# nitishthatte/QuadrotorILQR

Measured on AMD Instinct MI355X. Metric: iLQR solves/sec (batch, 100-knot SE(3) quadrotor), higher is better.
Workload: dtype f64

## Files before the change

### quadrotorilqr_amd/csrc/host/api_calls.h

```cpp
#pragma once

extern "C" {
int qilqr_solve_batch_device(qilqr_solver *s, const double *d_init, const double *d_desired_batch, int32_t B,
                             int32_t n, double *d_out_traj, double *d_out_cost, int32_t *d_out_status,
                             int32_t *d_out_iters, int32_t *d_out_n_bwd, int32_t *d_out_n_fwd) {
  return solve_batch_device_impl(s, d_init, d_desired_batch, B, n, d_out_traj, d_out_cost, d_out_status, d_out_iters,
                                 d_out_n_bwd, d_out_n_fwd, true);
}

int qilqr_stream_wait_event(qilqr_solver *s, void *hip_event) {
  if (!s || !hip_event) return fail(QILQR_ERR_INVALID_ARG, "null argument");
  HIP_TRY(hipSetDevice(s->device));
  HIP_TRY(hipStreamWaitEvent(s->stream, (hipEvent_t)hip_event, 0));
  return QILQR_OK;
}

namespace {
bool pinned_or_null(const void *p) {
  if (!p) return true;
  hipPointerAttribute_t a;
  if (hipPointerGetAttributes(&a, p) != hipSuccess) {
    (void)hipGetLastError();
    return false;
  }
// ... 68 lines not shown
    if (out_traj) e = hipMemcpyAsync(out_traj, s->stage_traj, tb, hipMemcpyDeviceToHost, s->stream);
    if (e == hipSuccess && out_cost) e = hipMemcpyAsync(out_cost, d_cost, sizeof(double) * B, hipMemcpyDeviceToHost, s->stream);
    if (e == hipSuccess && out_status) e = hipMemcpyAsync(out_status, d_int, sizeof(int) * B, hipMemcpyDeviceToHost, s->stream);
    if (e == hipSuccess && out_iters) e = hipMemcpyAsync(out_iters, d_int + B, sizeof(int) * B, hipMemcpyDeviceToHost, s->stream);
    if (e == hipSuccess && out_n_bwd) e = hipMemcpyAsync(out_n_bwd, d_int + 2 * B, sizeof(int) * B, hipMemcpyDeviceToHost, s->stream);
    if (e == hipSuccess && out_n_fwd) e = hipMemcpyAsync(out_n_fwd, d_int + 3 * B, sizeof(int) * B, hipMemcpyDeviceToHost, s->stream);
    if (e == hipSuccess) e = hipStreamSynchronize(s->stream);
    if (e == hipSuccess) e = hipGetLastError();
  }
  if (s->dev.profile) drain_events(s);
  if (e != hipSuccess) return fail(QILQR_ERR_HIP, std::string("copy back: ") + hipGetErrorString(e));
  return device_error(s);
}

void *qilqr_host_alloc(size_t bytes) {
  void *p = nullptr;
  if (hipHostMalloc(&p, bytes ? bytes : 1, hipHostMallocDefault) != hipSuccess) {
    g_last_error = "hipHostMalloc failed";
    return nullptr;
  }
  return p;
}
void qilqr_host_free(void *p) {
  if (p) (void)hipHostFree(p);
}

int qilqr_solve(qilqr_solver *s, const double *init, int32_t n, double *out_traj, double *out_cost,
                int32_t *out_status, int32_t *out_iters, double *debug_cost, double *debug_trajs,
                int32_t debug_cap, int32_t *n_debug) {
  if (!s || !init || !out_traj) return fail(QILQR_ERR_INVALID_ARG, "null argument");
  if (n <= 0) return fail(QILQR_ERR_INVALID_ARG, "empty trajectory");
  int rc;
  if ((rc = check_quaternions(init, n, "initial trajectory"))) return rc;
  if ((rc = begin_batch(s, 1, n, nullptr, E_SOLVE))) return rc;
  if ((rc = upload_tiled(s, init, s->st.traj[0], 1, n, 18))) return rc;
  const bool want_debug = s->options.populate_debug && debug_cap > 0 && (debug_cost || debug_trajs);
  if (want_debug) {
    const size_t want_t = debug_trajs ? (size_t)debug_cap * n * 18 : 0, want_c = (size_t)debug_cap;
    if (want_t > s->dbg_traj_cap) {
      if (s->dbg_trajs) (void)hipFree(s->dbg_trajs);
      s->dbg_trajs = nullptr;
      s->dbg_traj_cap = 0;
      HIP_TRY(hipMalloc((void **)&s->dbg_trajs, sizeof(double) * want_t));
      s->dbg_traj_cap = want_t;
    }
    if (want_c > s->dbg_cost_cap) {
      if (s->dbg_cost) (void)hipFree(s->dbg_cost);
      s->dbg_cost = nullptr;
      s->dbg_cost_cap = 0;
      HIP_TRY(hipMalloc((void **)&s->dbg_cost, sizeof(double) * want_c));
      s->dbg_cost_cap = want_c;
    }
    if (!s->dbg_seen) HIP_TRY(hipMalloc((void **)&s->dbg_seen, sizeof(int)));
    HIP_TRY(hipMemsetAsync(s->dbg_seen, 0, sizeof(int), s->stream));
    s->st.dbg_trajs = debug_trajs ? s->dbg_trajs : nullptr;
    s->st.dbg_cost = s->dbg_cost;
    s->st.dbg_seen = s->dbg_seen;
    s->st.dbg_cap = (int)debug_cap;
  }
  struct DebugRingScope {
    qilqr_solver *s;
    ~DebugRingScope() { s->st.dbg_trajs = s->st.dbg_cost = nullptr; s->st.dbg_seen = nullptr; s->st.dbg_cap = 0; }
  } ring_scope{s};
  auto capture = [&]() -> int {
    if (!want_debug || s->round_captured) return QILQR_OK;
    if (s->f32)
      launch(s, K_OTHER, k_debug_capture<float>, dim3(1), dim3(256), s->st, (int)n, debug_trajs ? s->dbg_trajs : nullptr, s->dbg_cost, s->dbg_seen, (int)debug_cap);
    else
// ... 118 lines not shown
```

### quadrotorilqr_amd/csrc/host/batch_solve.h

```cpp
#pragma once

namespace {
constexpr int MAX_TRACKED_DEVICES = 64;
std::atomic<int> g_solves_in_flight[MAX_TRACKED_DEVICES];
struct InFlight {
  std::atomic<int> &n;
  explicit InFlight(int device) : n(g_solves_in_flight[(unsigned)device % MAX_TRACKED_DEVICES]) { n.fetch_add(1, std::memory_order_relaxed); }
  ~InFlight() { n.fetch_sub(1, std::memory_order_relaxed); }
  bool alone(bool always = false) const { return always || n.load(std::memory_order_relaxed) == 1; }
};

int wait_for_count(const unsigned long long *word, hipStream_t stream, long old, unsigned long long *v) {
  const unsigned tag = (unsigned)((old & 0x3fffffff) + 1);
  for (long spins = 0;; ++spins) {
    *v = __atomic_load_n(word, __ATOMIC_ACQUIRE);
    if ((unsigned)(*v >> 32) == tag) return QILQR_OK;
    if ((spins & 1023) == 1023) {
      const hipError_t q = hipStreamQuery(stream);
      if (q != hipErrorNotReady) {
        *v = __atomic_load_n(word, __ATOMIC_ACQUIRE);
        if ((unsigned)(*v >> 32) == tag) return QILQR_OK;
        return fail(QILQR_ERR_HIP, std::string("a round never reported its active count: ") + hipGetErrorString(q));
      }
    }
// ... 62 lines not shown

int fire_early_out(qilqr_solver *s, long B, long n, EarlyOut *eo, unsigned active) {
  eo->fired = true;
  eo->late_cap = (int)active;
  *eo->layout = late_layout((long)active, n);
  int *early = s->d_early, *late_count = (int *)(s->d_late + eo->layout->count);
  launch(s, K_OTHER, k_mark_final, dim3(cdiv(B, 256)), dim3(256), s->st, (int)B, early, late_count);
  HIP_TRY(hipEventRecord(s->early_evt, s->stream));
  HIP_TRY(hipStreamWaitEvent(s->early_stream, s->early_evt, 0));
  hipStream_t main_stream = s->stream;
  s->stream = s->early_stream;
  int *d_int = s->stage_int;
  const int rc = gather(s, B, n, eo->h_traj ? s->stage_traj : nullptr, eo->h_cost ? s->stage_cost : nullptr, eo->h_status ? d_int : nullptr,
                        eo->h_iters ? d_int + B : nullptr, eo->h_bwd ? d_int + 2 * B : nullptr, eo->h_fwd ? d_int + 3 * B : nullptr, early, 1,
                        nullptr);
  s->stream = main_stream;
  if (rc) return rc;
  hipStream_t es = s->early_stream;
  if (eo->h_traj) HIP_TRY(hipMemcpyAsync(eo->h_traj, s->stage_traj, sizeof(double) * 18 * (size_t)B * n, hipMemcpyDeviceToHost, es));
  if (eo->h_cost) HIP_TRY(hipMemcpyAsync(eo->h_cost, s->stage_cost, sizeof(double) * B, hipMemcpyDeviceToHost, es));
  if (eo->h_status) HIP_TRY(hipMemcpyAsync(eo->h_status, d_int, sizeof(int) * B, hipMemcpyDeviceToHost, es));
  if (eo->h_iters) HIP_TRY(hipMemcpyAsync(eo->h_iters, d_int + B, sizeof(int) * B, hipMemcpyDeviceToHost, es));
  if (eo->h_bwd) HIP_TRY(hipMemcpyAsync(eo->h_bwd, d_int + 2 * B, sizeof(int) * B, hipMemcpyDeviceToHost, es));
  if (eo->h_fwd) HIP_TRY(hipMemcpyAsync(eo->h_fwd, d_int + 3 * B, sizeof(int) * B, hipMemcpyDeviceToHost, es));
  HIP_TRY(hipEventRecord(s->early_done, es));
  return QILQR_OK;
}

template <typename F>
int run_solve(qilqr_solver *s, long B, long n, int sync_every, F on_round, bool drain = true,
              const std::function<int(unsigned)> *on_count = nullptr, bool double_ok = false) {
  int rc;
  s->round_captured = false;
  if ((rc = launch_linearize(s, B, n, 0, 0))) return rc;
  {
    launch(s, K_OTHER, k_init, dim3(cdiv(B, 64)), dim3(64), s->params, s->st, (int)B, (int)n);
  }
  if (!(0.0 < s->params.max_iters)) {
    HIP_TRY(hipStreamSynchronize(s->stream));
    return QILQR_OK;
  }
  const double bound = (std::fmin(s->params.max_iters, 1e7) + 1.0) * ((double)std::max(s->params.ls_max_iters, 1) + 1.0) * (1.0 + max_restarts(s->params));
  const long max_rounds = (long)std::fmin(bound, 2e9);
  const int lag = (sync_every > 1) ? std::min(sync_every, 6) : 0;
  if (lag == 0) {
    for (long round = 0; round < max_rounds; ++round) {
      if ((rc = launch_backward(s, B, n, 0))) return rc;
      int active = 0;
      if ((rc = read_active(s, &active))) return rc;
      if ((rc = on_round())) return rc;
      if (active == 0) break;
      if ((rc = launch_rollout(s, B, n, F_SEARCH, round))) return rc;
      if ((rc = launch_linearize(s, B, n, 1, F_SEARCH))) return rc;
    }
  } else {
    struct CounterSet {
      qilqr_solver *s;
      int *base;
      CounterSet(qilqr_solver *s_, long round, bool two) : s(s_), base(s_->st.counters) { if (two) s->st.counters = base + (round & 1) * COUNT_WORDS; }
      ~CounterSet() { s->st.counters = base; }
    };
    for (int k = 0; k < 8; ++k) s->h_active[k] = 0;
    const InFlight in_flight(s->device);
    const bool can_fuse = s->route.combined && !s->compact;
    const TailFuse tf = tail_fuse(s->route, s->compact, 1);
    if (s->compact) s->plan_heads.push_back(0);
    unsigned seen_active = (unsigned)B;
    long used = B;
    bool pending_publish = false;
    unsigned launched_rounds[8] = {1, 1, 1, 1, 1, 1, 1, 1};
    bool two_sets = false;
    bool tail_started = false;
    for (long round = 0; round < max_rounds; ++round) {
      const RoctxRange range(s, "round", round);
      const bool compacting = s->compact && !tail_started && (seen_active > tf.stop || (tf.kinds && used > tf.slots));
      if (s->compact && tf.kinds && !compacting && used <= tf.slots && round >= tf.from) tail_started = true;
      s->live_hint = (long)seen_active;
      const bool fuse_now = (can_fuse || tail_started) && in_flight.alone(s->dev.fuse_in_flight == 1);
      if (fuse_now && s->route.round_kernel) {
        const RoundForm f = round_form(s->route, (can_fuse || tail_started) && double_ok, true, seen_active, used);
        if ((rc = launch_round(s, used, n, round, pending_publish, f.rounds, f.six))) return rc;
        s->round_captured = true;
        launched_rounds[round & 7] = f.rounds;
        pending_publish = true;
        two_sets = true;
        if ((rc = on_round())) return rc;
        goto round_enqueued;
      }
      if (pending_publish) {
        launch(s, K_OTHER, k_publish_active, dim3(1), dim3(64), s->st.counters + ((round + 1) & 1) * COUNT_WORDS, s->st.host_active,
               (int)((round - 1) & 0x3fffffff));
        pending_publish = false;
      }
      launched_rounds[round & 7] = 1;
      s->round_captured = false;
      {
      const CounterSet counter_set(s, round, two_sets);
      if (fuse_now) {
        if ((rc = launch_backward_rollout(s, used, n))) return rc;
      } else {
        if ((rc = launch_backward(s, used, n, 0))) return rc;
        if (compacting) {
          if ((rc = launch_compact(s, used, n))) return rc;
          used = slots_in_use(used, seen_active);
        }
        if ((rc = launch_rollout(s, used, n, F_SEARCH, round))) return rc;
      }
      if ((rc = on_round())) return rc;
      if ((rc = launch_linearize(s, used, n, 1, F_SEARCH, (int)(round & 0x3fffffff)))) return rc;
      }
    round_enqueued:
      if (round >= lag) {
        const long old = round - lag;
        unsigned long long v;
        if ((rc = wait_for_count(&s->h_active[old & 7], s->stream, old, &v))) return rc;
        if ((unsigned)v == 0) break;
        const unsigned now_at_most = ((unsigned)v + launched_rounds[old & 7] - 1) / launched_rounds[old & 7];
        seen_active = now_at_most;
        if (__atomic_load_n(s->h_active + 8 * (1 + qilqr_solver::MAX_PARTS), __ATOMIC_ACQUIRE)) {
          (void)hipStreamSynchronize(s->stream);
          if (s->early_stream) (void)hipStreamSynchronize(s->early_stream);
          return device_error(s);
        }
        if (on_count && (rc = (*on_count)(now_at_most))) return rc;
      }
    }
  }
  if (drain) {
    HIP_TRY(hipStreamSynchronize(s->stream));
    HIP_TRY(hipGetLastError());
    return device_error(s);
  }
  return QILQR_OK;
}

struct Part {
  hipStream_t stream;
  BatchState st;
  long nb;
  unsigned long long *h_active;
  bool done;
  unsigned seen_active;
  long used;
  bool tail = false;
  bool round_kernel = false;
  unsigned launched_rounds[8] = {1, 1, 1, 1, 1, 1, 1, 1};
};
BatchState slice_state(const qilqr_solver *s, long b0, long n, int part) {
  const BatchState &w = s->st;
  BatchState v = w;
  const size_t es = s->f32 ? sizeof(float) : sizeof(double);
  auto adv = [&](const void *p, long elems) { return (void *)((char *)p + (size_t)elems * es); };
  for (int k = 0; k < 2; ++k) {
    v.traj[k] = adv(w.traj[k], knot_base<true>(b0, n, 18));
    v.lin[k] = adv(w.lin[k], rec_base(w.layout, b0, n));
    v.knot_cost[k] = w.knot_cost[k] + cost_index(b0, 0, n);
  }
  v.gains = adv(w.gains, knot_base<true>(b0, n, 52));
  if (w.desired_tiled) v.desired = adv(w.desired, knot_base<true>(b0, n, 18));
  v.cur = w.cur + b0; v.cost = w.cost + b0; v.prev_cost = w.prev_cost + b0; v.terms = w.terms + 2 * b0;
// ... 95 lines not shown
        if ((rc = launch_rollout(s, part.used, n, F_SEARCH, round))) return rc;
        if ((rc = launch_linearize(s, part.used, n, 1, F_SEARCH, (int)(round & 0x3fffffff)))) return rc;
      }
      if (round < lag) continue;
      const long old = round - lag;
      for (auto &part : parts) {
        if (part.done) continue;
        unsigned long long v;
        if ((rc = wait_for_count(&part.h_active[old & 7], part.stream, old, &v))) return rc;
        part.seen_active = ((unsigned)v + part.launched_rounds[old & 7] - 1) / part.launched_rounds[old & 7];
        if ((unsigned)v == 0) {
          part.done = true;
          --remaining;
        }
      }
      if (__atomic_load_n(s->h_active + 8 * (1 + qilqr_solver::MAX_PARTS), __ATOMIC_ACQUIRE)) {
        for (auto &part : parts) (void)hipStreamSynchronize(part.stream);
        return device_error(s);
      }
    }
  }
  for (int p = 0; p < nparts; ++p) {
    HIP_TRY(hipEventRecord(s->part_done[p], parts[p].stream));
    HIP_TRY(hipStreamWaitEvent(s->stream, s->part_done[p], 0));
  }
  return QILQR_OK;
}

int solve_batch_device_impl(qilqr_solver *s, const double *d_init, const double *d_desired_batch, int32_t B, int32_t n,
                            double *d_out_traj, double *d_out_cost, int32_t *d_out_status, int32_t *d_out_iters,
                            int32_t *d_out_n_bwd, int32_t *d_out_n_fwd, bool drain) {
  if (!s || !d_init) return fail(QILQR_ERR_INVALID_ARG, "null argument");
  const RoctxRange range(s, "batch solve, trajectories:", (long)B);
  int rc = begin_batch(s, B, n, d_desired_batch, E_BATCH);
  if (rc) return rc;
  const bool persistent = s->route.persistent;
  if ((rc = to_tiled(s, d_init, s->st.traj[0], B, n, 18, persistent ? s->st.counters : nullptr))) return rc;
  const int nparts = s->route.parts;
  s->compact = s->route.compact;
  s->compact_out = CompactOut{d_out_traj, d_out_cost, d_out_status, d_out_iters, d_out_n_bwd, d_out_n_fwd};
  s->plan_heads.clear();
  struct CompactScope {
    qilqr_solver *s;
    ~CompactScope() { s->compact = false; }
  } compact_scope{s};
  if (persistent) {
    if ((rc = launch_solve4(s, B, n))) return rc;
  } else if (nparts > 1) {
    if ((rc = run_solve_parts(s, B, n, nparts))) return rc;
  } else {
    EarlyOut *eo = static_cast<EarlyOut *>(s->early_out);
    const std::function<int(unsigned)> hook = [&](unsigned active) -> int {
      if (eo->fired || active > eo->threshold) return QILQR_OK;
      return fire_early_out(s, B, n, eo, active);
    };
    if ((rc = run_solve(s, B, n, s->dev.sync_every, [] { return QILQR_OK; }, false, eo ? &hook : nullptr, true))) return rc;
    if (eo && eo->fired && eo->direct) {
      HIP_TRY(hipStreamWaitEvent(s->stream, s->early_done, 0));
      return gather(s, B, n, eo->v_traj, eo->v_cost, eo->v_status, eo->v_iters, eo->v_bwd, eo->v_fwd, s->d_early, 0, nullptr);
    }
    if (eo && eo->fired) {
      const LateLayout L = *eo->layout;
      int *early = s->d_early, *late_slot = early + s->early_cap, *late_idx = (int *)(s->d_late + L.idx), *late_count = (int *)(s->d_late + L.count);
      launch(s, K_OTHER, k_late_slots, dim3(cdiv(B, 256)), dim3(256), (int)B, (const int *)early, late_count, late_idx, late_slot, eo->late_cap);
      int *li = (int *)(s->d_late + L.ints);
      const long R = eo->late_cap;
      if ((rc = gather(s, B, n, eo->h_traj ? (double *)(s->d_late + L.traj) : nullptr, eo->h_cost ? (double *)(s->d_late + L.cost) : nullptr,
                       eo->h_status ? li : nullptr, eo->h_iters ? li + R : nullptr, eo->h_bwd ? li + 2 * R : nullptr,
                       eo->h_fwd ? li + 3 * R : nullptr, early, 0, late_slot)))
        return rc;
// ... 58 lines not shown
```

### quadrotorilqr_amd/csrc/host/describe.h

```cpp
#pragma once

extern "C" {
int qilqr_describe(qilqr_solver *s, int32_t B, char *buf, size_t cap) {
  if (!s || !buf || cap == 0 || B <= 0) return fail(QILQR_ERR_INVALID_ARG, "bad argument");
  const Route r = plan_route(route_inputs(s), B, CallFacts{s->dev.sync_every});
  std::string t;
  const bool persistent = r.persistent;
  const BackwardKind kind = persistent ? BW_FOUR : r.backward;
  if (kind == BW_ONE && !r.symmetric)
    t += "arithmetic: the reference's own forms (ilqr.hh:126-133: Eigen's diagonally pivoted LDL^T, V_x = Q_x - K^T Q_uu k, V_xx = Q_xx - K^T Q_uu K, "
         "not symmetrised)";
  else
    t += "arithmetic: symmetric-weight forms (Q == Q^T and R == R^T exactly: unpivoted LDL^T, V_x = Q_x + K^T Q_u, V_xx = Q_xx + Q_xu K on a symmetric "
         "accumulator; force_general = 1 selects the reference's own forms)";
  t += s->integrator == 1 ? "; Runge-Kutta step (extension)" : "; explicit Euler step (the reference's)";
  if (s->limited) {
    char lim[256];
    std::snprintf(lim, sizeof lim, "; control limits [lo, hi] (extension): lo = {%g, %g, %g, %g}, hi = {%g, %g, %g, %g} N, box QP per knot",
                  s->limits.lo[0], s->limits.lo[1], s->limits.lo[2], s->limits.lo[3], s->limits.hi[0], s->limits.hi[1], s->limits.hi[2], s->limits.hi[3]);
    t += lim;
  }
  if (s->modeled)
    t += "; per-problem models (extension): " + std::to_string(s->models_B) + " problems, each with its own mass, g, inertia and moment arms" +
         (B != s->models_B ? " (a call of B = " + std::to_string(B) + " problems is refused)" : std::string());
// ... 15 lines not shown
  t += s->f32 ? "; mixed precision (fp32 storage and lane-local arithmetic, fp64 recursion and cost sums)" : "; fp64";
  t += "; backward: ";
  t += persistent ? "k_solve4 (one launch per solve)" : kind == BW_FUSED ? "k_backward4, fused matrix + gradient wavefronts" : kind == BW_FOUR ? "k_backward4, six wavefronts"
       : kind == BW_TWO ? "k_backward2" : r.backward_ext.models ? std::string("k_backward_models<") + (r.symmetric ? "true>" : "false>") +
                                                        (r.backward_ext.limits ? " box form" : "") + ", one wavefront per trajectory"
       : r.backward_ext.limits ? "k_backward<true> box form, one wavefront per trajectory"
       : (r.symmetric ? "k_backward<true>, one wavefront per trajectory" : "k_backward<false>, one wavefront per trajectory (general kernel)");
  if (kind == BW_FOUR || backward_now(r, B) != kind)
    t += kind == BW_FOUR ? " (Q_uu factored by the gradient wavefront in launches with " + std::to_string(GFAC_MIN_LIVE) + " or more running trajectories, by the matrix wavefronts otherwise: the same bits)"
                         : " (six wavefronts, Q_uu factored by the gradient wavefront, while " + std::to_string(GFAC_MIN_LIVE) + " or more trajectories run: the same bits)";
  if (!persistent) {
    t += "; rollout: ";
    t += r.rollout == RO_LANE ? "k_rollout" : r.rollout == RO_16 ? "k_rollout16"
         : r.rollout == RO_THREE_THEN_16 ? "k_rollout3 for a trajectory's first " + std::to_string(ROLLOUT16_FROM) + " rollouts, k_rollout16 from there on" : "k_rollout3";
    const bool fused = r.combined && s->dev.sync_every > 1;
    const int parts = r.parts;
    const bool compact = r.compact;
    if (fused && parts == 1 && !compact)
      t += r.round_kernel ? "; round: one launch (k_round), " + std::to_string(r.rounds_per_launch) + " rounds per launch, while no other batch solve of the process is in flight on the device"
                          : std::string("; round: k_backward_rollout + k_linearize");
    else if (compact && r.fuse_kinds)
      t += "; round: three launches while the compaction runs, then " +
           std::string(r.linearize_ext.obstacles ? "k_backward_rollout + k_linearize (obstacles)" : "k_round (the mixed mode: k_backward_rollout + k_linearize)") +
           " once the running trajectories fit " + std::to_string(std::min(parts, 3)) + " block(s) of four per CU";
    else if (compact && r.compaction != 1 && r.late_tail)
      t += "; round: three launches, then " +
           std::string(r.linearize_ext.obstacles ? "k_backward_rollout + k_linearize (the same bits; obstacles)" : "k_round (the same bits; the mixed mode: k_backward_rollout + k_linearize)") +
           " once the running trajectories fit " + std::to_string(std::min(parts, 3)) + " block(s) of four per CU"
           + (r.late_from > 0 ? " and the rollouts are k_rollout16's (round " + std::to_string(r.late_from) + " on)" : std::string());
    else
      t += "; round: three launches";
    t += "; sub-batch streams: " + std::to_string(parts);
    t += compact ? "; compaction of the running trajectories: on (device-resident calls)" : "; compaction: off";
  }
  std::snprintf(buf, cap, "%s", t.c_str());
  return QILQR_OK;
}

int qilqr_compaction_moves(qilqr_solver *s, int64_t *moves) {
  if (!s || !moves) return fail(QILQR_ERR_INVALID_ARG, "null argument");
  HIP_TRY(hipSetDevice(s->device));
  HIP_TRY(hipStreamSynchronize(s->stream));
  *moves = 0;
  for (long head : s->plan_heads) {
    int m = 0;
    HIP_TRY(hipMemcpy(&m, s->st.plan + head + 2, sizeof(int), hipMemcpyDeviceToHost));
    *moves += m;
  }
  return QILQR_OK;
}

#if defined(QILQR_STAMPS) || defined(QILQR_ROUND_STAMPS)
int qilqr_debug_stamps(qilqr_solver *s, unsigned long long *out, int32_t B) {
  HIP_TRY(hipSetDevice(s->device));
  HIP_TRY(hipStreamSynchronize(s->stream));
  HIP_TRY(hipMemcpy(out, s->st.stamps, sizeof(unsigned long long) * 8 * B, hipMemcpyDeviceToHost));
  return QILQR_OK;
}
#endif

#ifdef QILQR_DIAG
int qilqr_debug_set_staged_late(int32_t on) {
  g_force_staged_late = on ? 1 : 0;
  return QILQR_OK;
}
int qilqr_debug_set_rollout_stall(qilqr_solver *s, int32_t knot) {
// ... 51 lines not shown
```

### quadrotorilqr_amd/csrc/host/launches.h

```cpp
#pragma once

namespace {
RouteInputs route_inputs(const qilqr_solver *s, bool models = true) {
  return RouteInputs{s->symmetric, s->q_diag, layout_kind(s->layout), s->f32, s->integrator, s->limited, s->modeled && models,
                     s->n_obstacles > 0 || s->pobs_B > 0, s->dev, s->num_cus, hw_queues(), s->pobs_B > 0};
}
enum Entry { E_BATCH, E_SOLVE, E_PASS, E_COST, E_SIM };
int refuse(const qilqr_solver *s, long B, Entry call) {
  if (call == E_BATCH && s->dev.persistent == 1) {
    if (s->limited) return fail(QILQR_ERR_INVALID_ARG, "control limits: persistent = 1 (k_solve4) has no box form; take the rounds (persistent = 0)");
    if (s->modeled)
      return fail(QILQR_ERR_INVALID_ARG, "batch models: persistent = 1 (k_solve4) has one model for the batch; take the rounds (persistent = 0)");
    if (s->n_obstacles > 0)
      return fail(QILQR_ERR_INVALID_ARG, "obstacles: persistent = 1 (k_solve4) linearises without them; take the rounds (persistent = 0)");
    if (s->pobs_B > 0)
      return fail(QILQR_ERR_INVALID_ARG, "batch obstacles: persistent = 1 (k_solve4) linearises without them; take the rounds (persistent = 0)");
  }
  if (call != E_SIM && s->pobs_B > 0 && B != s->pobs_B)
    return fail(QILQR_ERR_INVALID_ARG, "batch obstacles were set for B = " + std::to_string(s->pobs_B) + " problems; this call has B = " +
                                           std::to_string(B) + " (set them again, or clear them, for another batch)");
  if (call == E_SOLVE && s->modeled)
    return fail(QILQR_ERR_INVALID_ARG, "batch models are set: qilqr_solve solves one problem with the handle's model; use qilqr_solve_batch, or "
                                       "clear the models");
  if (call != E_COST && s->modeled && B != s->models_B)
    return fail(QILQR_ERR_INVALID_ARG, "batch models were set for B = " + std::to_string(s->models_B) + " problems; this call has B = " +
                                           std::to_string(B) + " (set them again, or clear them, for another batch)");
  return QILQR_OK;
}
int begin_batch(qilqr_solver *s, long B, long n, const double *d_desired_batch, Entry call) {
  if (B <= 0 || n <= 0) return fail(QILQR_ERR_INVALID_ARG, "B and n must be positive");
  if (!d_desired_batch && n > s->n_desired)
    return fail(QILQR_ERR_LENGTH_MISMATCH, "trajectory longer than desired trajectory");
  int rc = refuse(s, B, call);
  if (rc) return rc;
  HIP_TRY(hipSetDevice(s->device));
  rc = ensure_workspace(s, B, n);
  if (rc) return rc;
  if (d_desired_batch) {
    if (!s->desired_tiled && (rc = dalloc_s(s, &s->desired_tiled, (size_t)tiled_count(s->cap_B, s->cap_n, 18)))) return rc;
    if ((rc = to_tiled(s, d_desired_batch, s->desired_tiled, B, n, 18))) return rc;
    s->st.desired = s->desired_tiled;
    s->st.desired_tiled = 1;
  } else {
    s->st.desired = s->d_desired;
    s->st.desired_tiled = 0;
  }
  s->total_B = B;
  s->live_hint = 0;
  const CallFacts facts{s->dev.sync_every, d_desired_batch != nullptr, s->st.cost_hist != nullptr, s->early_out != nullptr, 0.0 < s->params.max_iters};
  s->route = plan_route(route_inputs(s, call != E_COST), B, facts);
  s->st.layout.tiled = s->route.tiled ? 1 : 0;
  launch(s, K_OTHER, k_begin, dim3(cdiv(B, 256)), dim3(256), s->st, (int)B);
  return QILQR_OK;
}

inline const ModelConsts<double> &consts_of(const qilqr_solver *s, double) { return s->consts; }
inline const ModelConsts<float> &consts_of(const qilqr_solver *s, float) { return s->constsf; }
template <typename S, int LK, int INTEG, bool TILED, typename... Ext>
int lin(qilqr_solver *s, long B, long n, int which, int need_flag, int round, Ext... ext) {
  const dim3 grid(cdiv(2 * ((B + 63) / 64) * 64 * n, QILQR_LIN_BLOCK));
  launch(s, K_LINEARIZE, (k_linearize<S, LK, INTEG, TILED, Ext...>), grid, dim3(QILQR_LIN_BLOCK), consts_of(s, S()),
         (const ModelConsts<S> *)s->d_consts, s->st, (int)B, (int)n, which, need_flag, round, ext...);
  return QILQR_OK;
}
template <int EXT>
auto lin_ext_args(const qilqr_solver *s, int which) {
  const BatchModels bm{s->d_models};
  const Obstacles ob{s->d_obstacles, s->n_obstacles};
  const ProblemObstacles po{ob, s->d_pobs, s->d_pobs_counts, s->pobs_K, (s->compact && which == 1) ? 1 : 0};
  if constexpr (EXT == LIN_PLAIN) return std::tuple<>();
  else if constexpr (EXT == LIN_MODELS) return std::make_tuple(bm);
  else if constexpr (EXT == LIN_OBSTACLES) return std::make_tuple(ob);
  else if constexpr (EXT == LIN_BOTH) return std::make_tuple(ModelsObstacles{bm, ob});
  else if constexpr (EXT == (LIN_OBSTACLES | LIN_PROBLEM)) return std::make_tuple(po);
  else return std::make_tuple(ModelsProblemObstacles{bm, po});
}
using LinLaunch = int (*)(qilqr_solver *, long, long, int, int, int);
template <int KEY>
int lin_keyed(qilqr_solver *s, long B, long n, int which, int need_flag, int round) {
  using S = std::conditional_t<(KEY >> 4) & 1, float, double>;
  return std::apply([&](auto... ext) { return lin<S, KEY & 3, (KEY >> 2) & 1, ((KEY >> 3) & 1) != 0>(s, B, n, which, need_flag, round, ext...); },
                    lin_ext_args<(KEY >> 5)>(s, which));
}
template <int KEY>
constexpr LinLaunch lin_launch() {
// ... 55 lines not shown
  return QILQR_OK;
}
int launch_rollout(qilqr_solver *s, long B, long n, int need_flag, long ordinal = -1) {
  auto ro = [&](auto kernel, dim3 grid, dim3 block, const auto &consts, auto... ext) {
    launch(s, K_ROLLOUT, kernel, grid, block, consts, s->st, (int)B, (int)n, need_flag, ext...);
  };
  const dim3 lanes(cdiv(B, 64)), fours(cdiv(B, 4));
  const Route &r = s->route;
  const ExtArgs &x = r.rollout_ext;
  if (r.rollout == RO_LANE && x.models) {
    const BatchModels bm{s->d_models};
    if (x.limits && r.integrator == 1) ro(k_rollout<double, 1, ControlLimits, BatchModels>, lanes, dim3(64), s->consts, s->limits, bm);
    else if (x.limits) ro(k_rollout<double, 0, ControlLimits, BatchModels>, lanes, dim3(64), s->consts, s->limits, bm);
    else if (r.integrator == 1) ro(k_rollout<double, 1, BatchModels>, lanes, dim3(64), s->consts, bm);
    else ro(k_rollout<double, 0, BatchModels>, lanes, dim3(64), s->consts, bm);
  } else if (r.rollout == RO_LANE && x.limits) {
    if (r.integrator == 1) ro(k_rollout<double, 1, ControlLimits>, lanes, dim3(64), s->consts, s->limits);
    else ro(k_rollout<double, 0, ControlLimits>, lanes, dim3(64), s->consts, s->limits);
  } else if (r.rollout == RO_LANE && r.integrator == 1) {
    ro(k_rollout<double, 1>, lanes, dim3(64), s->consts);
  } else if (r.rollout == RO_LANE) {
    if (s->f32) ro(k_rollout<float, 0>, lanes, dim3(64), s->constsf);
    else ro(k_rollout<double, 0>, lanes, dim3(64), s->consts);
  } else if (rollout16_now(r, ordinal)) {
    if (s->f32) ro(k_rollout16<float>, fours, dim3(192), s->consts);
    else ro(k_rollout16<double>, fours, dim3(192), s->consts);
  } else {
    if (s->f32) ro(k_rollout3<float>, lanes, dim3(192), s->constsf);
    else ro(k_rollout3<double>, lanes, dim3(192), s->consts);
  }
  return QILQR_OK;
}

int launch_round(qilqr_solver *s, long B, long n, long round, bool publish_prev, int rounds, bool six = false) {
  const ModelConsts<double> *cp = (const ModelConsts<double> *)s->d_consts;
  if (rounds == 2) six = false;
  const dim3 grid(cdiv(B, 4)), block(six ? 384 : 320);
  BatchState st = s->st;
  int *base = s->st.counters;
  st.counters = base + (round & 1) * COUNT_WORDS;
  int *prev = base + ((round + 1) & 1) * COUNT_WORDS;
  const int prev_round = publish_prev ? (int)((round - 1) & 0x3fffffff) : -1;
  const int lk = std::max(s->route.lin_kind, 1);
#define QILQR_LAUNCH_ROUND(LK, R, SIX)                                                                                                          \
  case LK * 16 + R * 2 + SIX:                                                                                                                     \
    launch(s, K_BACKWARD, (k_round<LK, R, SIX>), grid, block, s->consts, cp, s->params, st, (int)B, (int)n, prev, prev_round);                    \
    break
  switch (lk * 16 + rounds * 2 + (six ? 1 : 0)) {
    QILQR_LAUNCH_ROUND(3, 4, true); QILQR_LAUNCH_ROUND(2, 4, true); QILQR_LAUNCH_ROUND(1, 4, true);
    QILQR_LAUNCH_ROUND(3, 1, true); QILQR_LAUNCH_ROUND(2, 1, true); QILQR_LAUNCH_ROUND(1, 1, true);
    QILQR_LAUNCH_ROUND(3, 4, false); QILQR_LAUNCH_ROUND(2, 4, false); QILQR_LAUNCH_ROUND(1, 4, false);
    QILQR_LAUNCH_ROUND(3, 2, false); QILQR_LAUNCH_ROUND(2, 2, false); QILQR_LAUNCH_ROUND(1, 2, false);
    QILQR_LAUNCH_ROUND(3, 1, false); QILQR_LAUNCH_ROUND(2, 1, false); QILQR_LAUNCH_ROUND(1, 1, false);
    default: return fail(QILQR_ERR_INVALID_ARG, "k_round: no instantiation for this launch");
  }
#undef QILQR_LAUNCH_ROUND
  return QILQR_OK;
}
int launch_backward_rollout(qilqr_solver *s, long B, long n) {
  auto br = [&](auto kernel) { launch(s, K_BACKWARD, kernel, dim3(cdiv(B, 4)), dim3(320), s->consts, s->params, s->st, (int)B, (int)n); };
  if (s->f32) br(k_backward_rollout<float>);
  else br(k_backward_rollout<double>);
  return QILQR_OK;
}
int launch_accept(qilqr_solver *s, long B, long n, int ls_only) {
  launch(s, K_OTHER, k_accept, dim3(cdiv(B, 64)), dim3(64), s->params, s->st, (int)B, (int)n,
                     ls_only);
  return QILQR_OK;
}

inline long slots_in_use(long bound, unsigned seen_active) {
  const long want = std::max<long>(64, ((long)seen_active + 63) / 64 * 64);
  return std::min(bound, want);
// ... 45 lines not shown
```

### quadrotorilqr_amd/csrc/host/solver.h

```cpp
#pragma once

namespace {
thread_local std::string g_last_error;

int fail(int code, const std::string &msg) {
  g_last_error = msg;
  return code;
}

#define HIP_TRY(expr)                                                                        \
  do {                                                                                       \
    hipError_t _e = (expr);                                                                  \
    if (_e != hipSuccess)                                                                    \
      return fail(QILQR_ERR_HIP, std::string(#expr) + ": " + hipGetErrorString(_e));         \
  } while (0)

enum Kind { K_BACKWARD = 0, K_ROLLOUT = 1, K_LINEARIZE = 2, K_OTHER = 3, K_SOLVE = 4, K_KINDS = 5 };

struct EventPair {
  hipEvent_t a, b;
  int kind;
};

}
// ... 12 lines not shown
  void *d_desired = nullptr;
  void *d_ctab = nullptr;
  void *d_consts = nullptr;
  bool f32 = false;
  int integrator = 0;
  bool limited = false;
  ControlLimits limits{};
  bool modeled = false;
  long models_B = 0;
  double *d_models = nullptr;
  int n_obstacles = 0;
  double *d_obstacles = nullptr;
  std::vector<double> obstacles;
  long pobs_B = 0;
  int pobs_K = 0, pobs_max = 0;
  bool pobs_moving = false;
  double *d_pobs = nullptr;
  int *d_pobs_counts = nullptr;
  ModelConsts<float> constsf;
  long cap_B = 0, cap_n = 0;
  int hist_cap = 0;
  BatchState st{};
  std::vector<void *> allocs;
  int *h_counters = nullptr;
  unsigned long long *h_active = nullptr;
  unsigned long long *d_active = nullptr;
  static constexpr int MAX_PARTS = qilqr::MAX_PARTS;
  hipStream_t part_stream[MAX_PARTS] = {};
  hipEvent_t part_done[MAX_PARTS] = {};
  hipEvent_t main_ready = nullptr;
  int *d_part_counters = nullptr;
  long total_B = 0;
  Route route;
  bool round_captured = false;
  long live_hint = 0;
  double *io_aos = nullptr;
  size_t io_cap = 0;
  void *desired_tiled = nullptr;
  double *stage_traj = nullptr, *stage_des = nullptr, *stage_cost = nullptr;
  int *stage_int = nullptr;
  size_t stage_traj_cap = 0, stage_des_cap = 0, stage_B_cap = 0;
  void *early_out = nullptr;
  hipStream_t early_stream = nullptr;
  hipEvent_t early_evt = nullptr;
  hipEvent_t early_done = nullptr;
  int *d_early = nullptr;
  size_t early_cap = 0;
  char *d_late = nullptr, *h_late = nullptr;
  size_t late_bytes = 0;
  double *dbg_trajs = nullptr, *dbg_cost = nullptr;
  int *dbg_seen = nullptr;
  size_t dbg_traj_cap = 0, dbg_cost_cap = 0;
  std::vector<EventPair> events;
  size_t events_used = 0;
  double prof_ms[K_KINDS] = {0, 0, 0, 0, 0};
  unsigned prof_seen[K_KINDS] = {0, 0, 0, 0, 0};
  int prof_n[K_KINDS] = {0, 0, 0, 0, 0};
  int num_cus = 256;
  bool compact = false;
  qilqr::CompactOut compact_out{};
  std::vector<long> plan_heads;
};

namespace {

struct Roctx {
// ... 246 lines not shown
```

### quadrotorilqr_amd/csrc/kernels_common.h

```cpp
#pragma once

#include <hip/hip_runtime.h>
#include <stdint.h>

#ifdef QILQR_DIAG
#define QILQR_WITH_SOLVE4 1
#define QILQR_WITH_BACKWARD2 1
#endif

#include <type_traits>

#include "backward_layout.h"
#include "rollout16.h"
#include "se3_math.h"

namespace qilqr {

constexpr int COUNT_BASE = 8, COUNT_STRIPES = 64, COUNT_WORDS = COUNT_BASE + COUNT_STRIPES;
constexpr int F_ACTIVE = 1;
constexpr int F_SEARCH = 2;

struct SolveParams {
  double step_update, reduction_frac, rtol, atol, max_iters;
  int ls_max_iters;
// ... 1 lines not shown
};

struct BatchState {
  void *traj[2];
  void *lin[2];
  RecLayout layout;
  double *knot_cost[2];
  void *gains;
  const void *desired;
  int desired_tiled;
  int *cur;
  double *cost;
  double *prev_cost;
  double *terms;
  double *alpha;
  double *mu;
  int *trial;
  int *flags;
  int *status, *iters, *n_bwd, *n_fwd;
  int *counters;
  unsigned long long *host_active;
  unsigned long long *host_error;
  double *cost_hist;
  int hist_cap;
  const void *ctab;
  void *dump;
  unsigned long long *stamps;
  int *orig;
  int row0;
  int *plan;
  double *dbg_trajs, *dbg_cost;
  int *dbg_seen;
  int dbg_cap;
};

__device__ __forceinline__ int *active_counter(const BatchState &st) {
  return st.counters + COUNT_BASE + (blockIdx.x & (COUNT_STRIPES - 1));
}

typedef double d4 __attribute__((ext_vector_type(4)));
template <typename S>
struct GA {
  typedef const S __attribute__((address_space(1))) *cptr;
  typedef S v2 __attribute__((ext_vector_type(2)));
  typedef v2 __attribute__((address_space(1))) *ptr2;
  typedef const v2 __attribute__((address_space(1))) *cptr2;
};

#ifdef QILQR_STAMPS
#define QSTAMP(slot)                                                                   \
  do {                                                                                 \
    unsigned long long _t;                                                             \
    __builtin_amdgcn_sched_barrier(0);                                                 \
    asm volatile("s_memtime %0\n\ts_waitcnt lgkmcnt(0)" : "=s"(_t)::"memory");        \
    __builtin_amdgcn_sched_barrier(0);                                                 \
    stamp_sum[slot] += _t - stamp_prev;                                                \
    stamp_prev = _t;                                                                   \
  } while (0)
#define QKEEP(x) asm volatile("" ::"v"(x))
#else
#define QSTAMP(slot) do { } while (0)
#define QKEEP(x) do { } while (0)
#endif

__device__ __forceinline__ int xcd_local_block(unsigned hw_block, unsigned ) { return (int)hw_block; }
__device__ __forceinline__ bool is_converged(const SolveParams &p, double cost, double new_cost) {
// ... 35 lines not shown
```

### quadrotorilqr_amd/csrc/round_kernels.h

```cpp
#pragma once

#include "backward4_kernel.h"
#include "rollout16_kernel.h"
#include "linearize_kernels.h"

namespace qilqr {

template <typename S>
__global__ __launch_bounds__(320) void k_backward_rollout(ModelConsts<double> c, SolveParams p, BatchState st, int B, int n) {
  {
    constexpr int WAVES = 5;
    constexpr bool FUSED = true, FREE = true, GFAC = false;
    (void)GFAC;
    const int force = 0;
    (void)WAVES;
#define BW4_RETURN goto backward_done
#include "backward4_body.inc"
#undef BW4_RETURN
  }
backward_done:
  __syncthreads();
  if (threadIdx.x >= 192) return;
  {
    const int need_flag = F_SEARCH;
// ... 15 lines not shown
    if (b >= B) continue;
    const int fl = st.flags[b], buf = st.cur[b] ^ which;
    if (need_flag && !(fl & need_flag)) continue;
    if (nl == 0) { l0 = b; u0 = buf; } else if (nl == 1) { l1 = b; u1 = buf; } else if (nl == 2) { l2 = b; u2 = buf; } else { l3 = b; u3 = buf; }
    ++nl;
  }
  if (nl == 0) return;
  const int per = nl * n, wt = (per + 63) >> 6;
  for (int t = wave; t < 2 * wt; t += nwaves) {
    const bool cost_half = t < wt;
    const int r = (cost_half ? t : t - wt) * 64 + lane;
    if (r >= per) continue;
    const int i = (nl == 1) ? r : (nl == 2) ? (r >> 1) : (nl == 3) ? r / 3 : (r >> 2);
    const int g = r - i * nl;
    const int b = (g == 0) ? l0 : (g == 1) ? l1 : (g == 2) ? l2 : l3;
    const int buf = (g == 0) ? u0 : (g == 1) ? u1 : (g == 2) ? u2 : u3;
    S pt[18];
    load_knot<true>((const S *)st.traj[buf] + knot_base<true>(b, n, 18), i, 18, pt);
    S *rec = (S *)st.lin[buf] + rec_base(st.layout, b, n) + rec_elem(st.layout, i, 0);
    if (!cost_half) {
      const TiledRecWriter<S> wd{rec};
      linearize_dynamics(c, pt, wd);
      wd.flush();
    } else {
      const TiledRecWriter<S> w{rec};
      S pd[18];
      if (st.desired_tiled) load_knot<true>((const S *)st.desired + knot_base<true>(b, n, 18), i, 18, pd);
      else load_knot<false>((const S *)st.desired, i, 18, pd);
      const S cost = linearize_cost<LK>(qr, qr + 144, pt, pd, w);
      w.flush();
      st.knot_cost[buf][cost_index(b, i, n)] = (double)cost;
    }
  }
}
template <typename S, int LK>
__device__ __forceinline__ void round_follow(R16Lds &sh, const ModelConsts<S> &c, const S *qr, const BatchState &st, int b, int bs, int buf, bool live,
                                             bool single, int n, int lane) {
  const int per_task = single ? 64 : R16_CHUNK;
  const int groups = (n + per_task - 1) / per_task, ntasks = 2 * groups;
  for (;;) {
    int t = 0;
    if (lane == 0) t = __hip_atomic_fetch_add(&sh.flags[R16_F_TASK], 1, __ATOMIC_RELAXED, __HIP_MEMORY_SCOPE_WORKGROUP);
    t = __builtin_amdgcn_readfirstlane(t);
    if (t >= ntasks) break;
    const bool cost_half = single ? (t < groups) : ((t & 1) == 0);
    const int k0 = (single ? (cost_half ? t : t - groups) : (t >> 1)) * per_task;
    const int need = single ? n : ((k0 + R16_CHUNK < n) ? k0 + R16_CHUNK : n);
    const int m0 = (need - 1) - ((need - 1) & 1), m1 = (need - 1) - (((need - 1) & 1) ^ 1);
    if (!(r16_flag_wait_relaxed(sh, R16_F_K0, m0 + 1, lane) && (m1 < 0 || r16_flag_wait_relaxed(sh, R16_F_K1, m1 + 1, lane)))) break;
    const int i = k0 + (single ? lane : (lane & 15));
    if (!(single || live) || i >= n) continue;
    const int bb = single ? bs : b;
    S pt[18];
    load_knot<true>((const S *)st.traj[buf] + knot_base<true>(bb, n, 18), i, 18, pt);
    S *rec = (S *)st.lin[buf] + rec_base(st.layout, bb, n) + rec_elem(st.layout, i, 0);
    if (!cost_half) {
      const TiledRecWriter<S> wd{rec};
      linearize_dynamics(c, pt, wd);
      wd.flush();
    } else {
      const TiledRecWriter<S> w{rec};
      S pd[18];
      if (st.desired_tiled) load_knot<true>((const S *)st.desired + knot_base<true>(bb, n, 18), i, 18, pd);
      else load_knot<false>((const S *)st.desired, i, 18, pd);
      const S cost = linearize_cost<LK>(qr, qr + 144, pt, pd, w);
      w.flush();
      st.knot_cost[buf][cost_index(bb, i, n)] = (double)cost;
    }
  }
}
__device__ __forceinline__ void publish_active(int *counters, unsigned long long *host_active, int round, int lane) {
  int act = counters[COUNT_BASE + lane];
  counters[COUNT_BASE + lane] = 0;
#pragma unroll
  for (int off = 32; off > 0; off >>= 1) act += __shfl_xor(act, off);
  if (lane == 0)
    __hip_atomic_store(&host_active[round & 7], ((unsigned long long)(unsigned)(round + 1) << 32) | (unsigned)act, __ATOMIC_RELEASE,
                       __HIP_MEMORY_SCOPE_SYSTEM);
}
__global__ void k_publish_active(int *counters, unsigned long long *host_active, int round) {
  publish_active(counters, host_active, round, threadIdx.x & 63);
}
template <int LK, int ROUNDS, bool SIX = false>
__global__ __launch_bounds__(SIX ? 384 : 320) void k_round(ModelConsts<double> c, const ModelConsts<double> *__restrict__ cp, SolveParams p, BatchState st, int B,
                                                int n, int *prev_counters, int prev_round) {
  typedef double S;
  __shared__ double qr_w[160];
  BW4_DECLARE_LDS
  __shared__ R16Lds sh;
#ifdef QILQR_ROUND_STAMPS
  __shared__ unsigned long long round_stamp_x0;
  unsigned long long rs_t0 = 0, rs_t1 = 0, rs_t2 = 0, rs_t3 = 0;
#endif
#define BW4_LDS_DECLARED
#define R16_LDS_DECLARED
#define BW4_CTAB_FILLED
  for (int k = threadIdx.x; k < 160; k += blockDim.x) qr_w[k] = (k < 144) ? cp->Q[k] : cp->R[k - 144];
  if (threadIdx.x < 64) r16_exp2_lds[threadIdx.x >> 4][threadIdx.x & 15] = Series<double>::exp2[threadIdx.x >> 4][threadIdx.x & 15];
  bw4_fill_ctab<S>(ring, st.ctab, SIX ? 384 : 320);
#define ROUND_BEHIND_BACKWARD \
  if (blockIdx.x == 0 && (threadIdx.x >> 6) == 4 && prev_round >= 0) publish_active(prev_counters, st.host_active, prev_round, threadIdx.x & 63);
#define ROUND_ID 0
#include "round_body.inc"
#undef ROUND_ID
#undef ROUND_BEHIND_BACKWARD
#define ROUND_BEHIND_BACKWARD
  if constexpr (ROUNDS > 1) {
#define ROUND_ID 1
#include "round_body.inc"
#undef ROUND_ID
  }
  if constexpr (ROUNDS > 2) {
#define ROUND_ID 2
#include "round_body.inc"
#undef ROUND_ID
#define ROUND_ID 3
#include "round_body.inc"
#undef ROUND_ID
  }
#undef ROUND_BEHIND_BACKWARD
#undef BW4_LDS_DECLARED
#undef R16_LDS_DECLARED
#undef BW4_CTAB_FILLED
}

}
```

### quadrotorilqr_amd/csrc/route.h

```cpp
#pragma once

#include <algorithm>

#include "../../include/quadrotor_ilqr.h"

namespace qilqr {

inline unsigned cdiv(long a, long b) { return (unsigned)((a + b - 1) / b); }

#ifndef QILQR_REGIME_B
#define QILQR_REGIME_B 4096
#endif
constexpr long REGIME_B = QILQR_REGIME_B;
constexpr long R16_MAX_B = REGIME_B;
#ifndef QILQR_ROLLOUT16_FROM
#define QILQR_ROLLOUT16_FROM 16
#endif
constexpr long ROLLOUT16_FROM = QILQR_ROLLOUT16_FROM;
constexpr int MAX_PARTS = 8;

#ifndef QILQR_GFAC_MIN_LIVE
#define QILQR_GFAC_MIN_LIVE 3072
#endif
constexpr long GFAC_MIN_LIVE = QILQR_GFAC_MIN_LIVE;
// ... 110 lines not shown
  r.round_kernel = d.round_launch == 0 && !in.f32 && !in.obstacles;
  r.rounds_per_launch = (d.rounds_per_launch == 1 || d.rounds_per_launch == 2) ? d.rounds_per_launch : 4;
  r.late_tail = QILQR_LATE_TAIL && plain && fg == 0 && B > R16_MAX_B && r.backward == BW_FOUR && (swr == 0 || swr == 3);
  r.late_from = r.late_tail && swr == 0 ? ROLLOUT16_FROM : 0;
  r.parts = call.sync_every > 1 ? auto_parts(in, B) : 1;
  r.compact = d.compaction >= 0 && call.sync_every > 1 && !r.persistent && !call.cost_hist && !call.desired_batch && !call.early_out && !in.modeled &&
              call.iterates && (d.compaction == 1 || (!r.combined && r.backward != BW_ONE && r.tiled));
  return r;
}


inline BackwardKind backward_now(const Route &r, long live) {
  return (r.backward == BW_FUSED && r.force_general == 0 && live >= GFAC_MIN_LIVE) ? BW_FOUR : r.backward;
}
inline bool gradient_factors(const Route &r, long live) {
  const int fg = r.force_general;
  return fg == 7 || (fg != 8 && (r.many || fg == 0) && live >= GFAC_MIN_LIVE);
}
inline bool rollout16_now(const Route &r, long ordinal) {
  return r.rollout == RO_16 || (r.rollout == RO_THREE_THEN_16 && ordinal >= ROLLOUT16_FROM);
}

struct RoundForm {
  int rounds;
  bool six;
};
inline RoundForm round_form(const Route &r, bool several, bool forced, unsigned seen_active, long used) {
  RoundForm f{several ? r.rounds_per_launch : 1, false};
  const bool sparse = f.rounds > 1 && 2L * (long)seen_active <= cdiv(used, 4) * 4L;
  f.six = forced ? (r.force_general == 8 || (r.force_general == 0 && sparse)) : sparse;
  return f;
}

struct TailFuse {
  bool kinds = false;
  long slots = 0;
  unsigned stop = 0;
  long from = 0;
};
inline TailFuse tail_fuse(const Route &r, bool compacting, int nparts) {
  TailFuse t;
  t.stop = r.compaction == 1 ? 0u : COMPACT_STOP;
  if (!compacting || r.compaction == 1) return t;
  t.kinds = r.fuse_kinds || r.late_tail;
  t.from = r.late_from;
  if (t.kinds) {
    t.slots = std::max<long>(64, std::min(nparts, 3) * 4L * r.num_cus / nparts / 64 * 64);
    t.stop = std::max<unsigned>(t.stop, (unsigned)t.slots);
  }
  return t;
}

enum { LIN_PLAIN, LIN_MODELS, LIN_OBSTACLES, LIN_BOTH, LIN_PROBLEM = 4 };
constexpr int LIN_KEYS = 256;
constexpr int lin_key(int lk, int integ, bool tiled, bool f32, int ext) { return lk + 4 * integ + 8 * tiled + 16 * f32 + 32 * ext; }
constexpr bool lin_instantiated(int lk, int integ, bool tiled, bool f32, int ext) {
  const bool models = ext & LIN_MODELS, obstacles = ext & LIN_OBSTACLES, problem = ext & LIN_PROBLEM;
  if (problem && !obstacles) return false;
  if (f32 && (lk == 3 || integ == 1 || ext != LIN_PLAIN)) return false;
  if (integ == 1 && (tiled || lk == 3)) return false;
  if (tiled && models) return false;
  if (tiled && obstacles && lk == 0) return false;
  return lk >= 0 && lk <= 3 && (integ == 0 || integ == 1) && ext >= 0 && ext < 8;
}
constexpr bool lin_instantiated(int key) { return lin_instantiated(key & 3, (key >> 2) & 1, (key >> 3) & 1, (key >> 4) & 1, key >> 5); }

// ... 2 lines not shown
```

Measured before the change: 224,600.

## Fold solve startup (begin, retile, linearize, init) into the first round kernel launch

When the route is combined, non-compacted, single-part and alone on the device, the separate start kernels (k_begin, to_tiled retile, k_linearize, k_init) are skipped. The first k_round launch instead retiles the input, linearises and computes the initial cost in each block, with the counters cleared by a memset. This removes several kernel launches and their serialisation at the start of each solve. In exchange it adds a runtime branch and a startup prologue to the round kernel, plus a fallback path when the conditions do not hold.

```diff
diff --git a/quadrotorilqr_amd/csrc/host/api_calls.h b/quadrotorilqr_amd/csrc/host/api_calls.h
--- a/quadrotorilqr_amd/csrc/host/api_calls.h
+++ b/quadrotorilqr_amd/csrc/host/api_calls.h
@@ -124,8 +124,12 @@
   if (n <= 0) return fail(QILQR_ERR_INVALID_ARG, "empty trajectory");
   int rc;
   if ((rc = check_quaternions(init, n, "initial trajectory"))) return rc;
-  if ((rc = begin_batch(s, 1, n, nullptr, E_SOLVE))) return rc;
-  if ((rc = upload_tiled(s, init, s->st.traj[0], 1, n, 18))) return rc;
+  if ((rc = begin_batch(s, 1, n, nullptr, E_SOLVE, true))) return rc;
+  if (s->start_planned) {
+    if ((rc = ensure_io(s, (size_t)n * 18))) return rc;
+    HIP_TRY(hipMemcpyAsync(s->io_aos, init, sizeof(double) * (size_t)n * 18, hipMemcpyHostToDevice, s->stream));
+    s->start_in = s->io_aos;
+  } else if ((rc = upload_tiled(s, init, s->st.traj[0], 1, n, 18))) return rc;
   const bool want_debug = s->options.populate_debug && debug_cap > 0 && (debug_cost || debug_trajs);
   if (want_debug) {
     const size_t want_t = debug_trajs ? (size_t)debug_cap * n * 18 : 0, want_c = (size_t)debug_cap;
diff --git a/quadrotorilqr_amd/csrc/host/batch_solve.h b/quadrotorilqr_amd/csrc/host/batch_solve.h
--- a/quadrotorilqr_amd/csrc/host/batch_solve.h
+++ b/quadrotorilqr_amd/csrc/host/batch_solve.h
@@ -118,10 +118,17 @@
               const std::function<int(unsigned)> *on_count = nullptr, bool double_ok = false) {
   int rc;
   s->round_captured = false;
-  if ((rc = launch_linearize(s, B, n, 0, 0))) return rc;
-  {
+  const InFlight in_flight(s->device);
+  bool start_in_launch = s->start_planned && sync_every > 1 && !s->compact && in_flight.alone(s->dev.fuse_in_flight == 1);
+  if (!start_in_launch) {
+    if (s->start_planned) {
+      launch(s, K_OTHER, k_begin, dim3(cdiv(B, 256)), dim3(256), s->st, (int)B);
+      if (s->start_in && (rc = to_tiled(s, s->start_in, s->st.traj[0], B, n, 18))) return rc;
+    }
+    if ((rc = launch_linearize(s, B, n, 0, 0))) return rc;
     launch(s, K_OTHER, k_init, dim3(cdiv(B, 64)), dim3(64), s->params, s->st, (int)B, (int)n);
   }
+  s->start_planned = false;
   if (!(0.0 < s->params.max_iters)) {
     HIP_TRY(hipStreamSynchronize(s->stream));
     return QILQR_OK;
@@ -147,7 +154,6 @@
       ~CounterSet() { s->st.counters = base; }
     };
     for (int k = 0; k < 8; ++k) s->h_active[k] = 0;
-    const InFlight in_flight(s->device);
     const bool can_fuse = s->route.combined && !s->compact;
     const TailFuse tf = tail_fuse(s->route, s->compact, 1);
     if (s->compact) s->plan_heads.push_back(0);
@@ -162,10 +168,11 @@
       const bool compacting = s->compact && !tail_started && (seen_active > tf.stop || (tf.kinds && used > tf.slots));
       if (s->compact && tf.kinds && !compacting && used <= tf.slots && round >= tf.from) tail_started = true;
       s->live_hint = (long)seen_active;
-      const bool fuse_now = (can_fuse || tail_started) && in_flight.alone(s->dev.fuse_in_flight == 1);
+      const bool fuse_now = start_in_launch || ((can_fuse || tail_started) && in_flight.alone(s->dev.fuse_in_flight == 1));
       if (fuse_now && s->route.round_kernel) {
         const RoundForm f = round_form(s->route, (can_fuse || tail_started) && double_ok, true, seen_active, used);
-        if ((rc = launch_round(s, used, n, round, pending_publish, f.rounds, f.six))) return rc;
+        if ((rc = launch_round(s, used, n, round, pending_publish, f.rounds, f.six, start_in_launch))) return rc;
+        start_in_launch = false;
         s->round_captured = true;
         launched_rounds[round & 7] = f.rounds;
         pending_publish = true;
@@ -212,6 +219,7 @@
       }
     }
   }
+  if (start_in_launch) return fail(QILQR_ERR_INVALID_ARG, "a solve planned to start in its first k_round launch launched none");
   if (drain) {
     HIP_TRY(hipStreamSynchronize(s->stream));
     HIP_TRY(hipGetLastError());
@@ -373,10 +381,11 @@
                             int32_t *d_out_n_bwd, int32_t *d_out_n_fwd, bool drain) {
   if (!s || !d_init) return fail(QILQR_ERR_INVALID_ARG, "null argument");
   const RoctxRange range(s, "batch solve, trajectories:", (long)B);
-  int rc = begin_batch(s, B, n, d_desired_batch, E_BATCH);
+  int rc = begin_batch(s, B, n, d_desired_batch, E_BATCH, true);
   if (rc) return rc;
   const bool persistent = s->route.persistent;
-  if ((rc = to_tiled(s, d_init, s->st.traj[0], B, n, 18, persistent ? s->st.counters : nullptr))) return rc;
+  if (s->start_planned) s->start_in = d_init;
+  else if ((rc = to_tiled(s, d_init, s->st.traj[0], B, n, 18, persistent ? s->st.counters : nullptr))) return rc;
   const int nparts = s->route.parts;
   s->compact = s->route.compact;
   s->compact_out = CompactOut{d_out_traj, d_out_cost, d_out_status, d_out_iters, d_out_n_bwd, d_out_n_fwd};
diff --git a/quadrotorilqr_amd/csrc/host/describe.h b/quadrotorilqr_amd/csrc/host/describe.h
--- a/quadrotorilqr_amd/csrc/host/describe.h
+++ b/quadrotorilqr_amd/csrc/host/describe.h
@@ -71,6 +71,10 @@
       t += "; round: three launches";
     t += "; sub-batch streams: " + std::to_string(parts);
     t += compact ? "; compaction of the running trajectories: on (device-resident calls)" : "; compaction: off";
+    t += start_in_round(r, CallFacts{s->dev.sync_every}, true, true)
+             ? "; start of a solve: inside its first k_round launch (the blocks tile, linearise and arm their own trajectories), while no other batch solve "
+               "of the process is in flight on the device"
+             : "; start of a solve: kernels of its own (k_begin, k_retile, k_linearize, k_init)";
   }
   std::snprintf(buf, cap, "%s", t.c_str());
   return QILQR_OK;
diff --git a/quadrotorilqr_amd/csrc/host/launches.h b/quadrotorilqr_amd/csrc/host/launches.h
--- a/quadrotorilqr_amd/csrc/host/launches.h
+++ b/quadrotorilqr_amd/csrc/host/launches.h
@@ -27,7 +27,7 @@
                                            std::to_string(B) + " (set them again, or clear them, for another batch)");
   return QILQR_OK;
 }
-int begin_batch(qilqr_solver *s, long B, long n, const double *d_desired_batch, Entry call) {
+int begin_batch(qilqr_solver *s, long B, long n, const double *d_desired_batch, Entry call, bool plain_start = false) {
   if (B <= 0 || n <= 0) return fail(QILQR_ERR_INVALID_ARG, "B and n must be positive");
   if (!d_desired_batch && n > s->n_desired)
     return fail(QILQR_ERR_LENGTH_MISMATCH, "trajectory longer than desired trajectory");
@@ -50,7 +50,9 @@
   const CallFacts facts{s->dev.sync_every, d_desired_batch != nullptr, s->st.cost_hist != nullptr, s->early_out != nullptr, 0.0 < s->params.max_iters};
   s->route = plan_route(route_inputs(s, call != E_COST), B, facts);
   s->st.layout.tiled = s->route.tiled ? 1 : 0;
-  launch(s, K_OTHER, k_begin, dim3(cdiv(B, 256)), dim3(256), s->st, (int)B);
+  s->start_in = nullptr;
+  s->start_planned = plain_start && start_in_round(s->route, facts, true, true);
+  if (!s->start_planned) launch(s, K_OTHER, k_begin, dim3(cdiv(B, 256)), dim3(256), s->st, (int)B);
   return QILQR_OK;
 }
 
@@ -172,13 +174,19 @@
   return QILQR_OK;
 }
 
-int launch_round(qilqr_solver *s, long B, long n, long round, bool publish_prev, int rounds, bool six = false) {
+int launch_round(qilqr_solver *s, long B, long n, long round, bool publish_prev, int rounds, bool six = false, bool start = false) {
   const ModelConsts<double> *cp = (const ModelConsts<double> *)s->d_consts;
   if (rounds == 2) six = false;
+  if (start) six = false;
   const dim3 grid(cdiv(B, 4)), block(six ? 384 : 320);
   BatchState st = s->st;
   int *base = s->st.counters;
   st.counters = base + (round & 1) * COUNT_WORDS;
+  if (start) {
+    HIP_TRY(hipMemsetAsync(base, 0, sizeof(int) * 2 * COUNT_WORDS, s->stream));
+    st.start = 1;
+    st.start_in = s->start_in;
+  }
   int *prev = base + ((round + 1) & 1) * COUNT_WORDS;
   const int prev_round = publish_prev ? (int)((round - 1) & 0x3fffffff) : -1;
   const int lk = std::max(s->route.lin_kind, 1);
diff --git a/quadrotorilqr_amd/csrc/host/solver.h b/quadrotorilqr_amd/csrc/host/solver.h
--- a/quadrotorilqr_amd/csrc/host/solver.h
+++ b/quadrotorilqr_amd/csrc/host/solver.h
@@ -68,6 +68,8 @@
   int *d_part_counters = nullptr;
   long total_B = 0;
   Route route;
+  bool start_planned = false;
+  const double *start_in = nullptr;
   bool round_captured = false;
   long live_hint = 0;
   double *io_aos = nullptr;
diff --git a/quadrotorilqr_amd/csrc/kernels_common.h b/quadrotorilqr_amd/csrc/kernels_common.h
--- a/quadrotorilqr_amd/csrc/kernels_common.h
+++ b/quadrotorilqr_amd/csrc/kernels_common.h
@@ -57,6 +57,8 @@
   double *dbg_trajs, *dbg_cost;
   int *dbg_seen;
   int dbg_cap;
+  int start;
+  const double *start_in;
 };
 
 __device__ __forceinline__ int *active_counter(const BatchState &st) {
diff --git a/quadrotorilqr_amd/csrc/round_kernels.h b/quadrotorilqr_amd/csrc/round_kernels.h
--- a/quadrotorilqr_amd/csrc/round_kernels.h
+++ b/quadrotorilqr_amd/csrc/round_kernels.h
@@ -71,6 +71,68 @@
       st.knot_cost[buf][cost_index(b, i, n)] = (double)cost;
     }
   }
+}
+template <int LK>
+__device__ __forceinline__ void round_start(const ModelConsts<double> &c, const double *qr, double (&ring)[4][4][BW2_BUF], const SolveParams &p,
+                                            const BatchState &st, int B, int n) {
+  typedef double S;
+  typedef typename GA<S>::v2 sv2;
+  const int lane = threadIdx.x & 63;
+  const int wave = __builtin_amdgcn_readfirstlane((int)(threadIdx.x >> 6));
+  const int b0 = (int)blockIdx.x * 4, nb = (B - b0 < 4) ? B - b0 : 4;
+  if (st.start_in) {
+    for (int q = threadIdx.x; q < 4 * n * 9; q += blockDim.x) {
+      const int g = q & 3, kp = q >> 2;
+      if (g >= nb) continue;
+      const int i = kp / 9, pr = kp - 9 * i;
+      const long b = b0 + g, pi = (b * n * 9 + kp) * 2;
+      const sv2 v = {st.start_in[pi], st.start_in[pi + 1]};
+      *reinterpret_cast<sv2 *>((S *)st.traj[0] + knot_base<true>(b, n, 18) + knot_elem<true>(i, 2 * pr, 18)) = v;
+    }
+  }
+  if ((int)threadIdx.x < nb) {
+    st.cur[b0 + threadIdx.x] = 0;
+    st.flags[b0 + threadIdx.x] = 0;
+  }
+  __syncthreads();
+  linearize_block<S, LK>(c, qr, st, b0, B, n, 0, 0);
+  __syncthreads();
+  if (wave < nb) {
+    const int b = b0 + wave;
+    const double *kc = st.knot_cost[0];
+    double *scr = &ring[wave][0][0];
+    double s = 0.0;
+    for (int base = 0; base < n; base += 64) {
+      const int i = base + lane, cnt = (n - base < 64) ? n - base : 64;
+      scr[lane] = (i < n) ? kc[cost_index(b, i, n)] : 0.0;
+      int t = 0;
+      for (; t + 8 <= cnt; t += 8) {
+        double x[8];
+#pragma unroll
+        for (int e = 0; e < 8; ++e) x[e] = scr[t + e];
+#pragma unroll
+        for (int e = 0; e < 8; ++e) s += x[e];
+      }
+      for (; t < cnt; ++t) s += scr[t];
+    }
+    if (lane == 0) {
+      st.cost[b] = s;
+      st.prev_cost[b] = s;
+      st.iters[b] = 0;
+      st.n_bwd[b] = 0;
+      st.n_fwd[b] = 0;
+      st.trial[b] = 0;
+      st.alpha[b] = 1.0;
+      st.mu[b] = 0.0;
+      st.terms[2 * b] = 0.0;
+      st.terms[2 * b + 1] = 0.0;
+      st.status[b] = 2;
+      st.flags[b] = (0.0 < p.max_iters) ? F_ACTIVE : 0;
+      if (st.orig) st.orig[b] = st.row0 + b;
+      if (b == 0 && st.plan) st.plan[2] = 0;
+    }
+  }
+  __syncthreads();
 }
 template <typename S, int LK>
 __device__ __forceinline__ void round_follow(R16Lds &sh, const ModelConsts<S> &c, const S *qr, const BatchState &st, int b, int bs, int buf, bool live,
@@ -137,6 +199,10 @@
   for (int k = threadIdx.x; k < 160; k += blockDim.x) qr_w[k] = (k < 144) ? cp->Q[k] : cp->R[k - 144];
   if (threadIdx.x < 64) r16_exp2_lds[threadIdx.x >> 4][threadIdx.x & 15] = Series<double>::exp2[threadIdx.x >> 4][threadIdx.x & 15];
   bw4_fill_ctab<S>(ring, st.ctab, SIX ? 384 : 320);
+#ifndef QILQR_EDGES_APART
+  if constexpr (!SIX)
+    if (st.start) round_start<LK>(c, qr_w, ring, p, st, B, n);
+#endif
 #define ROUND_BEHIND_BACKWARD \
   if (blockIdx.x == 0 && (threadIdx.x >> 6) == 4 && prev_round >= 0) publish_active(prev_counters, st.host_active, prev_round, threadIdx.x & 63);
 #define ROUND_ID 0
diff --git a/quadrotorilqr_amd/csrc/route.h b/quadrotorilqr_amd/csrc/route.h
--- a/quadrotorilqr_amd/csrc/route.h
+++ b/quadrotorilqr_amd/csrc/route.h
@@ -166,6 +166,16 @@
   return f;
 }
 
+inline bool start_in_round(const Route &r, const CallFacts &call, bool plain_input, bool alone) {
+#ifdef QILQR_EDGES_APART
+  (void)r; (void)call; (void)plain_input; (void)alone;
+  return false;
+#else
+  return r.combined && r.round_kernel && !r.f32 && !r.compact && r.parts == 1 && !r.persistent && call.sync_every > 1 && call.iterates && plain_input &&
+         alone;
+#endif
+}
+
 struct TailFuse {
   bool kinds = false;
   long slots = 0;
```

Result: no change. 224,200 (-0.2%).
